# syb0rg/qwen3-tts-jetson

Hardware: AMD Instinct MI355X
Metric: audio frames/sec (12 Hz frames) + RTF, Qwen3-TTS-0.6B batch=1 and batch=8xN (higher is better)
Workload: dtype f16; 1 GPU; configs[1]: Qwen3-TTS-0.6B 1 utterance(s)/GPU x 512 frames, talker+code-predictor+vocoder(full) HIP path, temp 0.9 top-k 50; utterances_per_gpu=1, frames=512, vocoder=full, parallelism=utterance-sharded dp1, weights=local GGUF read

## Files before the change

qwen3-tts-jetson_amd/csrc/persist_cp.hip:

```cpp
#include "persist.h"
#include "persist_dev.h"
#ifdef Q3T_DEV
namespace q3t { __device__ uint64_t *g_selprof = nullptr; }
#define SEL_STAMP(k)                                                                                              \
    do {                                                                                                          \
        if (threadIdx.x == 0 && q3t::g_selprof)                                                                   \
            q3t::g_selprof[((size_t)blockIdx.x * PROF_PH + 440 + ((k) >> 2)) * 4 + ((k) & 3)] = wall_clock64();   \
    } while (0)
#endif
#include "select.h"

#pragma clang fp contract(off)
#include "persist_roles.h"

#ifndef Q3T_CP_SGATE
#define Q3T_CP_SGATE 1
#endif
#ifndef Q3T_CP_GATE
#define Q3T_CP_GATE 1
#endif
#ifndef Q3T_CP_WPUB
#define Q3T_CP_WPUB 1
#endif
#ifndef Q3T_CP_PUT_FIRST
// ... 76 lines not shown
#if Q3T_CP_PAIR
#define CP_TOKENS(pass, ps) for (int ps = (pass) == 1 ? 0 : (pass); ps <= (pass); ++ps)
#else
#define CP_TOKENS(pass, ps) if (const int ps = (pass); true)
#endif
__device__ __forceinline__ int ph_of(int pass, int l, int k) { return pass * PPH + 5 * l + k; }
__device__ __forceinline__ int next_layer(int pass, int l) {
    if (pass + 1 == NPASS && l + 1 == NLC) return -1;
    return (l + 1 < NLC && !(pass == 0 && l + 1 == NLC - 1)) ? l + 1 : 0;
}

__device__ __forceinline__ void role_qkv(Ctx &X) {
    const PersistParams &p = X.p;
    CLds &S = X.S;
    const int i = blockIdx.x - QW, t = threadIdx.x, grp = t >> 4;
    const float temp = p.sel.temperature;
    const bool samp = temp > 0.0f && Q3T_CP_RANGE;
    uint4 wq[4][8];
    float4 nw;
    auto issue_qkv = [&](int l) { qkv_issue<Pol>(S.layers[l].qkv, S.layers[l].attn_norm, i, wq, nw); };
    issue_qkv(0);
    for (int pass = PAIR ? 1 : 0; pass < NPASS; ++pass) {
        for (int l = 0; l < NLC; ++l)
        CP_TOKENS(pass, ps) {
            if (ps >= 1 && l == 0) continue;
            X.use(ps);
            const int ph = ph_of(ps, l, 0);
            float4 x;
            if (l == 0) {
                x = ldf4(p.x_in + 4 * t);
            } else {
                uint32_t u[4];
                PROF(ph, 0);
                wait_in<Pol, 4>(X, p.gx + 4 * t, X.tag(ph_of(ps, l - 1, 4)), u);
                PROF(ph, 1);
                x = f4_of(u);
            }
            qkv_phase<Pol>(X, i, x, wq, nw, ph);
            if (ps < pass && l > 0) continue;
            if (l + 1 < NLC) {
                issue_qkv(l + 1);
            } else if (pass >= 1) {
#pragma unroll
                for (int j = 0; j < 2; ++j) issue_row(S.heads[pass - 1], 32 * i + 16 * j + grp, wq[j]);
                nw = ldf4(p.out_norm + 4 * t);
            } else {
                issue_qkv(1);
            }
        }
        if (pass == 0) continue;
        const int hph = ph_of(pass, NLC, 0);
        uint32_t u[4];
        PROF(hph, 0);
        wait_in<Pol, 4>(X, p.gx + 4 * t, X.tag(ph_of(pass, NLC - 1, 4)), u);
        PROF(hph, 1);
        rms_to_f16(f4_of(u), nw, p.eps, S.xs, S.dscr, nullptr);
        __syncthreads();
        head_rows<2>(X, wq);
        __syncthreads();
        PROF(hph, 3);
        if (t < 64) {
            const float lg = S.outv[t & 31];
            const float sv = samp && Q3T_CP_PREDIV ? lg / temp : lg;
            const float mx = group_max<32>(sv), mn = -group_max<32>(sv > -INFINITY ? -sv : -INFINITY);
            if (t < 32 || (samp && t < 34))
                g_put(t < 32 ? p.glog + 32 * i + t : p.glog + CPV + MMS * i + (t - 32),
                      __float_as_uint(t < 32 ? sv : t == 32 ? mx : mn), X.tag(hph));
            if (t < 32) p.logits[32 * i + t] = lg;
        }
        published<Pol>(X, hph);
        if (pass + 1 < NPASS) issue_qkv(1);
    }
}

__device__ __forceinline__ void role_att(Ctx &X) {
    const PersistParams &p = X.p;
    CLds &S = X.S;
    const int g = blockIdx.x - AW, t = threadIdx.x, lane = t & 63, wave = t >> 6;
    const int pg = t >> 4, li = t & 15;
    const int hb = wave == 0 ? g * 256 : wave == 1 ? g * 256 + D : wave == 2 ? NH * D + g * D : (NH + NKV) * D + g * D;
    const int gi = hb + lane;
    for (int e = t; e < NLC * D; e += 256) {
        S.qn[e / D][e % D] = S.layers[e / D].qn[e % D];
        S.kn[e / D][e % D] = S.layers[e / D].kn[e % D];
    }
    for (int e = t; e < 16 * D; e += 256) S.rope[e / D][e % D] = p.rope[e];
    S.sel.hist[t] = 0u;
// ... 99 lines not shown
                    v16[n] = v16[n + 1] = 0.0f;
                    fma2(pr[n >> 3], ok ? v8[n & 7] : 0.0f, ok ? v8[(n + 1) & 7] : 0.0f, v16[n], v16[n + 1]);
                }
#pragma unroll
                for (int m = 0; m < 8; ++m) {
                    const auto sw = __builtin_amdgcn_permlane16_swap(__float_as_uint(v16[2 * m]), __float_as_uint(v16[2 * m + 1]), false, false);
                    c8[m] = __uint_as_float((uint32_t)sw[0]) + __uint_as_float((uint32_t)sw[1]);
                }
#pragma unroll
                for (int q = 0; q < 4; ++q) {
                    const auto sw = __builtin_amdgcn_permlane32_swap(__float_as_uint(c8[2 * q]), __float_as_uint(c8[2 * q + 1]), false, false);
                    const float av = __uint_as_float((uint32_t)sw[0]) + __uint_as_float((uint32_t)sw[1]);
                    const int n = 4 * q + (lane >> 4);
                    S.ared[wave][n >> 3][li * 8 + (n & 7)] = av;
                }
            }
            __syncthreads();
            if (t < 128) {
                const int h = t / (D / 2), d = 2 * (t % (D / 2));
                const float lsum = (S.wsum[0][h] + S.wsum[1][h]) + (S.wsum[2][h] + S.wsum[3][h]);
                const float a0 = (S.ared[0][h][d] + S.ared[1][h][d]) + (S.ared[2][h][d] + S.ared[3][h][d]);
                const float a1 = (S.ared[0][h][d + 1] + S.ared[1][h][d + 1]) + (S.ared[2][h][d + 1] + S.ared[3][h][d + 1]);
                g_put(p.gattn + g * 128 + t, (uint32_t)f2h(a0 / lsum) | ((uint32_t)f2h(a1 / lsum) << 16), X.tag(ph));
            }
            PROF(ph, 2);
        }
        if (pass == 0) continue;
        const int hph = ph_of(pass, NLC, 0);
        const bool samp = p.sel.temperature > 0.0f;
        constexpr bool RNG = Q3T_CP_RANGE;
        const float u = uniform24(spre.seed, spre.utt, (uint64_t)spre.frame, (uint64_t)pass);
        uint32_t u8[8], mm[2];
        PROF(hph, 0);
        if (Q3T_CP_SGATE) g_gate(p.glog + 8 * t, X.tag(hph), X.c);
        if constexpr (Q3T_POLL16) {
            if (samp && RNG) g_wait16_pair<8, 2>(p.glog + 8 * t, p.glog + CPV + MMS * lane, X.tag(hph), u8, mm, X.c);
            else g_waitc<8>(p.glog + 8 * t, X.tag(hph), u8, X.c);
        } else {
            if (samp && RNG) g_wait_pair<8, 2>(p.glog + 8 * t, p.glog + CPV + MMS * lane, X.tag(hph), u8, mm, X.c);
            else g_wait<8>(p.glog + 8 * t, X.tag(hph), u8, X.c);
        }
        PROF(hph, 1);
        float v[SEL_VPT_MAX];
#pragma unroll
        for (int e = 0; e < SEL_VPT_MAX; ++e) v[e] = e < 8 ? __uint_as_float(u8[e]) : -INFINITY;
        SelectSpec sp = p.sel;
        sp.step = pass - 1;
        int sel;
        if (spre.done >= 0) {
            sel = -1;
        } else if (!samp) {
            sel = sel_argmax(v, CPV, 8, S.sel);
        } else if (!RNG) {
            sel = select_token_pre<SEL_CP>(sp, spre, v, S.sel);
        } else {
            float mx = wave_max(__uint_as_float(mm[0])), mn = -wave_max(-__uint_as_float(mm[1]));
            if constexpr (!Q3T_CP_PREDIV) {
#pragma unroll
                for (int e = 0; e < 8; ++e) v[e] = v[e] / p.sel.temperature;
                mx = mx / p.sel.temperature;
                mn = mn / p.sel.temperature;
            }
            sel = sel_sample_range(v, CPV, 8, p.sel.top_k, u, mx, mn, S.sel);
        }
        S.sel.hist[t] = 0u;
        PROF(hph, 3);
        if (g == 0 && t == 0) {
            if (pass + 1 < NPASS) g_put(p.gtok + pass, (uint32_t)max(sel, 0), X.tag(hph));
            if (sel >= 0) select_commit(sp, 0, sel);
            if (pass + 1 == NPASS) __hip_atomic_store(p.seq, X.seq + 1u, __ATOMIC_RELAXED, __HIP_MEMORY_SCOPE_AGENT);
        }
// ... 23 lines not shown
    };
    issue(0);
    int it = 0;
    for (int pass = PAIR ? 1 : 0; pass < NPASS; ++pass) {
        for (int l = 0; l < NLC; ++l)
        CP_TOKENS(pass, ps) {
            if (ps == 0 && l == NLC - 1) continue;
            X.use(ps);
            const int par = it++ & 1;
            const int ph = ph_of(ps, l, 2);
            if (t < 32) {
                const int row = 32 * i + t;
                float xr;
                if (l == 0 && ps == 0) {
                    xr = p.x_in[row];
                } else if (l == 0) {
                    int tok = p.gs.tok[0];
                    if (pass >= 2) {
                        uint32_t u1[1];
                        g_wait<1>(p.gtok + pass - 1, X.tag(ph_of(pass - 1, NLC, 0)), u1, X.c);
                        tok = min((int)u1[0], p.sel.V - 1);
                    }
                    xr = p.xtab ? p.xtab[((size_t)(pass == 1 ? 0 : VOC + (pass - 2) * CPV) + tok) * H + row]
                                : h2f(S.tabs[pass - 1][(size_t)tok * H + row]);
                } else {
                    uint32_t u1[1];
                    g_wait<1>(p.gx + row, X.tag(ph_of(ps, l - 1, 4)), u1, X.c);
                    xr = __uint_as_float(u1[0]);
                }
                S.xr[t] = xr;
            }
            uint32_t u[4];
            PROF(ph, 0);
            wait_in<Pol, 4>(X, p.gattn + 4 * t, X.tag(ph_of(ps, l, 1)), u);
            PROF(ph, 1);
            *reinterpret_cast<uint4 *>(S.xs + 8 * t) = make_uint4(u[0], u[1], u[2], u[3]);
            wave_lds_sync();
            float acc[8];
#pragma unroll
            for (int j = 0; j < 8; ++j) {
                acc[j] = 0.0f;
#pragma unroll
                for (int tt = 0; tt < 4; ++tt)
                    acc[j] = dot8(wo[j][tt], *reinterpret_cast<const uint4 *>(S.xs + wave * 512 + l16 * 8 + tt * 128), acc[j]);
            }
#pragma unroll
            for (int j = 0; j < 8; ++j) {
                acc[j] = group_sum<16>(acc[j]);
                if (l16 == 0) S.red[par][wave][4 * j + grp4] = acc[j];
            }
            __syncthreads();
            if (t < 32) {
                const float (&rd)[4][32] = S.red[par];
                const float s = rd[0][t] + rd[1][t] + rd[2][t] + rd[3][t];
                g_put(p.gx2 + 32 * i + t, __float_as_uint(S.xr[t] + s), X.tag(ph));
            }
            published<Pol>(X, ph);
            if (ps == pass && next_layer(pass, l) >= 0) issue(next_layer(pass, l));
        }
    }
}

__device__ __forceinline__ void role_gu(Ctx &X) {
    const PersistParams &p = X.p;
    CLds &S = X.S;
    const int i = blockIdx.x - UW, t = threadIdx.x;
    uint4 wg[2][8], wu[2][8];
    float4 nw;
    gu_issue(S.layers[0].gu, S.layers[0].ffn_norm, i, wg, wu, nw);
    for (int pass = PAIR ? 1 : 0; pass < NPASS; ++pass) {
        for (int l = 0; l < NLC; ++l)
        CP_TOKENS(pass, ps) {
            if (ps == 0 && l == NLC - 1) continue;
            X.use(ps);
            const int ph = ph_of(ps, l, 3);
            uint32_t u[4];
            PROF(ph, 0);
            wait_in<Pol, 4>(X, p.gx2 + 4 * t, X.tag(ph_of(ps, l, 2)), u);
            PROF(ph, 1);
            gu_phase<Pol>(X, i, f4_of(u), wg, wu, nw, ph);
            const int nl = ps == pass ? next_layer(pass, l) : -1;
            if (nl >= 0) gu_issue(S.layers[nl].gu, S.layers[nl].ffn_norm, i, wg, wu, nw);
        }
    }
}

__device__ __forceinline__ void role_dn(Ctx &X) {
    const PersistParams &p = X.p;
    CLds &S = X.S;
    const int i = blockIdx.x - DW, t = threadIdx.x;
    const int lo = i * H / ND, n = (i + 1) * H / ND - lo;
    uint4 wd[5][6];
    dn_issue(S.layers[0].down, lo, n, wd);
    int it = 0;
    for (int pass = PAIR ? 1 : 0; pass < NPASS; ++pass) {
        for (int l = 0; l < NLC; ++l)
        CP_TOKENS(pass, ps) {
            if (ps == 0 && l == NLC - 1) continue;
            X.use(ps);
            if (t < n) {
                uint32_t u1[1];
                g_wait<1>(p.gx2 + lo + t, X.tag(ph_of(ps, l, 2)), u1, X.c);
                S.xr[t] = __uint_as_float(u1[0]);
            }
            dn_phase<Pol>(X, lo, n, it++ & 1, wd, ph_of(ps, l, 4));
            const int nl = ps == pass ? next_layer(pass, l) : -1;
            if (nl >= 0) dn_issue(S.layers[nl].down, lo, n, wd);
        }
    }
}

__global__ void __launch_bounds__(256) k_cp_roles(const PersistParams p) {
    extern __shared__ __attribute__((aligned(16))) uint8_t smem[];
    CLds &S = *reinterpret_cast<CLds *>(smem);
    const int t = threadIdx.x, w = blockIdx.x;
    Ctx X{p, p, S, Ctl{p.err, false}, __hip_atomic_load(p.seq, __ATOMIC_RELAXED, __HIP_MEMORY_SCOPE_AGENT)};
#ifdef Q3T_DEV
    if (w == 0 && t == 0) g_selprof = p.prof;
#endif
    if (t < NLC) S.layers[t] = p.L[t];
    if (t < 15) S.heads[t] = p.heads[t];
    if (t < 16) S.tabs[t] = p.gs.tabs[t];
    __syncthreads();
    if (w < AW) role_qkv(X);
    else if (w < OW) role_att(X);
    else if (w < UW) role_o(X);
    else if (w < DW) role_gu(X);
    else role_dn(X);
}

size_t cp_roles_lds() { return std::max(sizeof(CLds), (size_t)96 * 1024); }

}

bool persist_cp_roles_resident(int device) {
    int n_cu = 0, blocks = 0;
    if (hipDeviceGetAttribute(&n_cu, hipDeviceAttributeMultiprocessorCount, device) != hipSuccess || n_cu < G) return false;
    const void *k = reinterpret_cast<const void *>(&k_cp_roles);
    if (hipFuncSetAttribute(k, hipFuncAttributeMaxDynamicSharedMemorySize, (int)cp_roles_lds()) != hipSuccess) return false;
    return hipOccupancyMaxActiveBlocksPerMultiprocessor(&blocks, k, 256, cp_roles_lds()) == hipSuccess && blocks >= 1;
}

bool persist_cp_roles(const PersistParams &p, hipStream_t s) {
    if (!p.L || p.n_layers != NLC || !p.heads || !p.logits || !p.rope || !p.x_in || !p.gs.tok || !p.gs.tabs || !p.qkvtab ||
        !p.gx || p.sel.mode != SEL_CP || p.sel.V != CPV) {
        set_error("persist_cp_roles: bad parameters");
        return false;
    }
    static bool attr = false;
    if (!attr) {
        Q3T_HIP(hipFuncSetAttribute(reinterpret_cast<const void *>(&k_cp_roles), hipFuncAttributeMaxDynamicSharedMemorySize,
                                    (int)cp_roles_lds()));
        attr = true;
    }
    hipLaunchKernelGGL(k_cp_roles, dim3(G), dim3(256), cp_roles_lds(), s, p);
    Q3T_HIP(hipGetLastError());
    return true;
}

}
```

qwen3-tts-jetson_amd/csrc/persist_dev.h:

```cpp
#pragma once
#include "persist.h"

namespace q3t {
namespace pdev {

constexpr unsigned SPIN_LIMIT = 1u << 21;
#ifndef Q3T_POLL_SLEEP
#define Q3T_POLL_SLEEP 1
#endif

template <class V>
__device__ __forceinline__ V ldgv(const void *p) {
    typedef const __attribute__((address_space(1))) V gV;
    return *(gV *)(p);
}
__device__ __forceinline__ uint4 ld16(const void *p) {
    const u32x4_t v = ldgv<u32x4_t>(p);
    return make_uint4(v.x, v.y, v.z, v.w);
}
__device__ __forceinline__ float4 ldf4(const float *p) {
    typedef float f4v __attribute__((ext_vector_type(4)));
    const f4v v = ldgv<f4v>(p);
    return make_float4(v.x, v.y, v.z, v.w);
}
__device__ __forceinline__ uint2 ld8(const void *p) {
    typedef unsigned u2v __attribute__((ext_vector_type(2)));
    const u2v v = ldgv<u2v>(p);
    return make_uint2(v.x, v.y);
}

__device__ __forceinline__ void g_put(uint64_t *p, uint32_t payload, uint32_t tag) {
    __hip_atomic_store(p, ((uint64_t)tag << 32) | payload, __ATOMIC_RELAXED, __HIP_MEMORY_SCOPE_AGENT);
}
__device__ __forceinline__ uint64_t g_ld(const uint64_t *p) {
    return __hip_atomic_load(p, __ATOMIC_RELAXED, __HIP_MEMORY_SCOPE_AGENT);
}
__device__ __forceinline__ uint4 ld16_sc1(const uint16_t *p) {
    uint64_t *q = reinterpret_cast<uint64_t *>(const_cast<uint16_t *>(p));
    const uint64_t a = __hip_atomic_load(q, __ATOMIC_RELAXED, __HIP_MEMORY_SCOPE_AGENT);
    const uint64_t b = __hip_atomic_load(q + 1, __ATOMIC_RELAXED, __HIP_MEMORY_SCOPE_AGENT);
    return make_uint4((uint32_t)a, (uint32_t)(a >> 32), (uint32_t)b, (uint32_t)(b >> 32));
}

struct Ctl {
    unsigned *err;
    bool abort;
};
__device__ __forceinline__ bool give_up(Ctl &c, unsigned &it) {
    if ((++it & 255u) == 0 && (__hip_atomic_load(c.err, __ATOMIC_RELAXED, __HIP_MEMORY_SCOPE_AGENT) != 0u || it >= SPIN_LIMIT)) {
        c.abort = true;
        __hip_atomic_fetch_or(c.err, 1u, __ATOMIC_RELAXED, __HIP_MEMORY_SCOPE_AGENT);
        return true;
    }
    return false;
}

template <int N, int STRIDE = 1, int RUN = 1>
__device__ __forceinline__ void g_wait(const uint64_t *base, uint32_t tag, uint32_t (&out)[N], Ctl &c) {
    uint64_t v[N];
    unsigned it = 0;
    while (true) {
#pragma unroll
        for (int i = 0; i < N; ++i) v[i] = g_ld(base + (i / RUN) * STRIDE + i % RUN);
        bool ok = true;
#pragma unroll
        for (int i = 0; i < N; ++i) ok &= (uint32_t)(v[i] >> 32) == tag;
        if (ok || c.abort) break;
        if (give_up(c, it)) break;
        if constexpr (Q3T_POLL_SLEEP > 0) __builtin_amdgcn_s_sleep(Q3T_POLL_SLEEP);
    }
#pragma unroll
    for (int i = 0; i < N; ++i) out[i] = (uint32_t)v[i];
}

#ifndef Q3T_POLL16
#define Q3T_POLL16 1
#endif
template <int M>
__device__ __forceinline__ void ld16_sc1_batch(const uint64_t *const (&a)[M], u32x4_t (&r)[M]) {
// ... 71 lines not shown
    else g_wait<N>(base, tag, out, c);
}

template <int N, int M>
__device__ __forceinline__ void g_wait_pair(const uint64_t *a, const uint64_t *b, uint32_t tag, uint32_t (&oa)[N], uint32_t (&ob)[M],
                                            Ctl &c) {
    uint64_t v[N + M];
    unsigned it = 0;
    while (true) {
#pragma unroll
        for (int i = 0; i < N; ++i) v[i] = g_ld(a + i);
#pragma unroll
        for (int i = 0; i < M; ++i) v[N + i] = g_ld(b + i);
        bool ok = true;
#pragma unroll
        for (int i = 0; i < N + M; ++i) ok &= (uint32_t)(v[i] >> 32) == tag;
        if (ok || c.abort) break;
        if (give_up(c, it)) break;
        if constexpr (Q3T_POLL_SLEEP > 0) __builtin_amdgcn_s_sleep(Q3T_POLL_SLEEP);
    }
#pragma unroll
    for (int i = 0; i < N; ++i) oa[i] = (uint32_t)v[i];
#pragma unroll
    for (int i = 0; i < M; ++i) ob[i] = (uint32_t)v[N + i];
}

__device__ __forceinline__ void g_gate(const uint64_t *g, uint32_t tag, Ctl &c) {
    if ((threadIdx.x & 63) == 0) {
        unsigned it = 0;
        while (!c.abort && (uint32_t)(g_ld(g) >> 32) != tag) {
            give_up(c, it);
            __builtin_amdgcn_s_sleep(1);
        }
    }
    c.abort = __shfl(c.abort ? 1 : 0, 0) != 0;
}
template <int N, int STRIDE = 1, int RUN = 1>
__device__ __forceinline__ void g_wait_gated(const uint64_t *base, uint32_t tag, uint32_t (&out)[N], Ctl &c) {
    g_gate(base, tag, c);
    g_wait<N, STRIDE, RUN>(base, tag, out, c);
}

#ifndef Q3T_WAVE_SYNC
#define Q3T_WAVE_SYNC 1
#endif
__device__ __forceinline__ void wave_lds_sync() {
    if constexpr (Q3T_WAVE_SYNC) {
        __builtin_amdgcn_s_waitcnt(0xc07f);
        __builtin_amdgcn_wave_barrier();
    } else {
        __syncthreads();
    }
}

__device__ __forceinline__ float4 f4_of(const uint32_t (&u)[4]) {
    return make_float4(__uint_as_float(u[0]), __uint_as_float(u[1]), __uint_as_float(u[2]), __uint_as_float(u[3]));
}


__device__ __forceinline__ double block_sum_d(double v, double *scr) {
    const int lane = threadIdx.x & 63, wave = threadIdx.x >> 6;
    v = wave_sum_d(v);
    if (lane == 0) scr[wave] = v;
    __syncthreads();
    return (scr[0] + scr[1]) + (scr[2] + scr[3]);
}

__device__ __forceinline__ void rms_to_f16(float4 x, float4 w, float eps, uint16_t *xs, double *dscr, float *side) {
    const int t = threadIdx.x;
    double ss = (double)(x.x * x.x) + (double)(x.y * x.y) + (double)(x.z * x.z) + (double)(x.w * x.w);
    ss = block_sum_d(ss, dscr);
    const float scale = 1.0f / sqrtf((float)(ss / 1024) + eps);
    const float y0 = (x.x * scale) * w.x, y1 = (x.y * scale) * w.y, y2 = (x.z * scale) * w.z, y3 = (x.w * scale) * w.w;
// ... 43 lines not shown
```

qwen3-tts-jetson_amd/csrc/persist_roles.h:

```cpp
#pragma once
#include "persist_dev.h"

#pragma clang fp contract(off)

namespace q3t {
namespace prole {
using namespace pdev;

constexpr int H = 1024, NH = 16, NKV = 8, D = 128, QKVN = (NH + 2 * NKV) * D, INTER = 3072;

template <class LDS>
struct RoleCtx {
    const PersistParams &p;
    LDS &S;
    Ctl c;
    unsigned seq;
    __device__ uint32_t tag(int ph) const { return ((seq * 1024u + (unsigned)ph) << 1) | 1u; }
};

#define PROF(ph, k)                                                                                           \
    do {                                                                                                      \
        if (X.p.prof && threadIdx.x == 0 && blockIdx.x < PROF_WG) X.p.prof[((size_t)blockIdx.x * PROF_PH + (ph)) * 4 + (k)] = wall_clock64(); \
    } while (0)

template <class P, int N, class C>
__device__ __forceinline__ void wait_in(C &X, const uint64_t *g, uint32_t tag, uint32_t (&u)[N]) {
    if (P::GATE) g_gate(g, tag, X.c);
    P::template wait<N>(g, tag, u, X.c);
}
template <class P, class C>
__device__ __forceinline__ void published(C &X, int ph) {
    PROF(ph, 2);
    if (P::PUT_FIRST) __syncthreads();
}

__device__ __forceinline__ void issue_row(const uint16_t *W, int row, uint4 (&w)[8]) {
    const uint16_t *r = W + (size_t)row * H + (threadIdx.x & 15) * 8;
#pragma unroll
    for (int tt = 0; tt < 8; ++tt) w[tt] = ld16(r + tt * 128);
}

template <class P>
__device__ __forceinline__ void qkv_issue(const uint16_t *W, const float *norm, int i, uint4 (&wq)[4][8], float4 &nw) {
    const int t = threadIdx.x, grp = t >> 4;
#pragma unroll
    for (int j = 0; j < 4; ++j)
        issue_row(W, 64 * i + (P::WPUB ? 16 * (t >> 6) + 4 * j + (grp & 3) : 16 * j + grp), wq[j]);
    nw = ldf4(norm + 4 * t);
}
template <class P, class C>
__device__ __forceinline__ void qkv_phase(C &X, int i, float4 x, const uint4 (&wq)[4][8], float4 nw, int ph) {
    auto &S = X.S;
    const int t = threadIdx.x, l16 = t & 15, grp = t >> 4;
    rms_to_f16(x, nw, X.p.eps, S.xs, S.dscr, nullptr);
    __syncthreads();
    float acc[4];
#pragma unroll
    for (int j = 0; j < 4; ++j) {
        acc[j] = 0.0f;
#pragma unroll
        for (int tt = 0; tt < 8; ++tt) acc[j] = dot8(wq[j][tt], *reinterpret_cast<const uint4 *>(S.xs + l16 * 8 + tt * 128), acc[j]);
// ... 64 lines not shown
        for (int tt = 0; tt < 4; ++tt) {
            const uint4 xv = *reinterpret_cast<const uint4 *>(S.xs + l16 * 8 + tt * 128);
            a0[j] = dot8(wg[j][tt], xv, a0[j]);
            b0[j] = dot8(wu[j][tt], xv, b0[j]);
        }
#pragma unroll
        for (int tt = 4; tt < 8; ++tt) {
            const uint4 xv = *reinterpret_cast<const uint4 *>(S.xs + l16 * 8 + tt * 128);
            a1[j] = dot8(wg[j][tt], xv, a1[j]);
            b1[j] = dot8(wu[j][tt], xv, b1[j]);
        }
    }
#pragma unroll
    for (int j = 0; j < 2; ++j) {
        const float ga = group_sum<16>(a0[j]) + group_sum<16>(a1[j]);
        const float ub = group_sum<16>(b0[j]) + group_sum<16>(b1[j]);
        if (l16 == 0) S.hs[16 * j + grp] = silu_f(ga) * ub;
    }
    __syncthreads();
    if (t < 16) g_put(X.p.gh + 16 * i + t, (uint32_t)f2h(S.hs[2 * t]) | ((uint32_t)f2h(S.hs[2 * t + 1]) << 16), X.tag(ph));
    published<P>(X, ph);
}

__device__ __forceinline__ void dn_issue(const uint16_t *W, int lo, int n, uint4 (&wd)[5][6]) {
    const int t = threadIdx.x, wave = t >> 6, grp4 = (t & 63) >> 4;
#pragma unroll
    for (int j = 0; j < 5; ++j) {
        const uint16_t *r = W + (size_t)(lo + min(4 * j + grp4, n - 1)) * INTER + wave * 768 + (t & 15) * 8;
#pragma unroll
        for (int tt = 0; tt < 6; ++tt) wd[j][tt] = ld16(r + tt * 128);
    }
}
template <class P, class C>
__device__ __forceinline__ void dn_phase(C &X, int lo, int n, int par, const uint4 (&wd)[5][6], int ph) {
    auto &S = X.S;
    const int t = threadIdx.x, wave = t >> 6, l16 = t & 15, grp4 = (t & 63) >> 4;
    uint32_t u[6];
    PROF(ph, 0);
    wait_in<P, 6>(X, X.p.gh + 6 * t, X.tag(ph - 1), u);
    PROF(ph, 1);
    *reinterpret_cast<uint2 *>(S.xs + 12 * t) = make_uint2(u[0], u[1]);
    *reinterpret_cast<uint2 *>(S.xs + 12 * t + 4) = make_uint2(u[2], u[3]);
    *reinterpret_cast<uint2 *>(S.xs + 12 * t + 8) = make_uint2(u[4], u[5]);
    wave_lds_sync();
    float acc[5];
#pragma unroll
    for (int j = 0; j < 5; ++j) {
        acc[j] = 0.0f;
#pragma unroll
        for (int tt = 0; tt < 6; ++tt)
            acc[j] = dot8(wd[j][tt], *reinterpret_cast<const uint4 *>(S.xs + wave * 768 + l16 * 8 + tt * 128), acc[j]);
    }
#pragma unroll
    for (int j = 0; j < 5; ++j) {
        acc[j] = group_sum<16>(acc[j]);
        if (l16 == 0) S.red[par][wave][4 * j + grp4] = acc[j];
    }
    __syncthreads();
    if (t < n) {
        const float (&rd)[4][32] = S.red[par];
        const float s = rd[0][t] + rd[1][t] + rd[2][t] + rd[3][t];
        g_put(X.p.gx + lo + t, __float_as_uint(S.xr[t] + s), X.tag(ph));
    }
    published<P>(X, ph);
}

}
}
```

qwen3-tts-jetson_amd/csrc/persist_tk.hip:

```cpp
#include "persist.h"
#include "persist_dev.h"
#include "select.h"

#include <algorithm>

#pragma clang fp contract(off)
#include "persist_roles.h"

namespace q3t {

namespace {
using namespace prole;

constexpr int VOC = 3072;
constexpr int R = NH / NKV, CHK = 64, PSLOT = 264, MAXCH = 32;
#ifndef Q3T_TK_WPUB
#define Q3T_TK_WPUB 1
#endif
#ifndef Q3T_TK_HOIST
#define Q3T_TK_HOIST 1
#endif
#ifndef Q3T_TK_PUT_FIRST
#define Q3T_TK_PUT_FIRST 0
#endif
// ... 178 lines not shown
            for (int tt = 0; tt < 4; ++tt) acc[j] = dot8(wo[j][tt], *reinterpret_cast<const uint4 *>(S.xs + l16 * 8 + tt * 128), acc[j]);
        }
#pragma unroll
        for (int j = 0; j < 8; ++j) {
            acc[j] = group_sum<16>(acc[j]);
            if (l16 == 0) S.outv[32 * wave + 4 * j + grp4] = acc[j];
        }
        __syncthreads();
        if (t < 128) g_put(p.gop + (size_t)w * H + 128 * rb + t, __float_as_uint(S.outv[t]), X.tag(ph));
        published<Pol>(X, ph);
        if (l + 1 < nl) issue(l + 1);
    }
}

__device__ __forceinline__ void tk_gu(Ctx &X) {
    const PersistParams &p = X.p;
    TLds &S = X.S;
    const int i = blockIdx.x - UW, t = threadIdx.x, nl = X.nl;
    uint4 wg[2][8], wu[2][8];
    float4 nw;
    gu_issue(S.layers[0].gu, S.layers[0].ffn_norm, i, wg, wu, nw);
    for (int l = 0; l < nl; ++l) {
        const int ph = 5 * l + 3;
        float4 xr;
        if (l == 0) {
            xr = gather_x4(p);
        } else {
            uint32_t u4[4];
            g_waitc<4>(p.gx + 4 * t, X.tag(5 * (l - 1) + 4), u4, X.c);
            xr = f4_of(u4);
        }
        uint32_t u[16];
        PROF(ph, 0);
        g_gate(p.gop + 4 * t, X.tag(5 * l + 2), X.c);
        if constexpr (Q3T_POLL16) g_wait16<4, 4, H>(p.gop + 4 * t, X.tag(5 * l + 2), u, X.c);
        else g_wait<16, H, 4>(p.gop + 4 * t, X.tag(5 * l + 2), u, X.c);
        PROF(ph, 1);
        float x[4];
#pragma unroll
        for (int e = 0; e < 4; ++e) {
            const float s = ((__uint_as_float(u[e]) + __uint_as_float(u[4 + e])) + __uint_as_float(u[8 + e])) + __uint_as_float(u[12 + e]);
            x[e] = (e == 0 ? xr.x : e == 1 ? xr.y : e == 2 ? xr.z : xr.w) + s;
        }
        gu_phase<Pol>(X, i, make_float4(x[0], x[1], x[2], x[3]), wg, wu, nw, ph);
        if (l + 1 < nl) gu_issue(S.layers[l + 1].gu, S.layers[l + 1].ffn_norm, i, wg, wu, nw);
    }
}

__device__ __forceinline__ void tk_dn(Ctx &X) {
    const PersistParams &p = X.p;
    TLds &S = X.S;
    const int i = blockIdx.x - DW, t = threadIdx.x, nl = X.nl;
    const int lo = i * H / ND, n = (i + 1) * H / ND - lo;
    uint4 wd[5][6];
    dn_issue(S.layers[0].down, lo, n, wd);
    for (int l = 0; l < nl; ++l) {
        if (t < n) {
            float xr;
            if (l == 0) {
                xr = layer0_x1(p, lo + t);
            } else {
                uint32_t u1[1];
                g_wait<1>(p.gx + lo + t, X.tag(5 * (l - 1) + 4), u1, X.c);
                xr = __uint_as_float(u1[0]);
            }
            uint32_t uo[4];
            g_wait<4, H>(p.gop + lo + t, X.tag(5 * l + 2), uo, X.c);
            const float s = ((__uint_as_float(uo[0]) + __uint_as_float(uo[1])) + __uint_as_float(uo[2])) + __uint_as_float(uo[3]);
            S.xr[t] = xr + s;
// ... 244 lines not shown
    PROF(hph, 1);
    if (p.sel.mode != SEL_NONE) {
        float v[SEL_VPT_MAX];
#pragma unroll
        for (int e = 0; e < SEL_VPT_MAX; ++e) v[e] = e < VOC / 256 ? __uint_as_float(u[e]) : -INFINITY;
        tok = select_token_pre<SEL_CB0>(p.sel, spre, v, S.sel);
    }
    __syncthreads();
    if (t == 0) {
        if (tok >= 0) select_commit(p.sel, 0, tok);
        if (p.adv_pos && !(p.adv_done && p.adv_done[0] >= 0)) {
            p.adv_pos[0] += 1;
            p.adv_frame[0] += 1;
        }
        __hip_atomic_store(p.seq, X.seq + 1u, __ATOMIC_RELAXED, __HIP_MEMORY_SCOPE_AGENT);
    }
    PROF(hph, 2);
}

__global__ void __launch_bounds__(256, 2) k_tk_roles(const PersistParams p) {
    extern __shared__ __attribute__((aligned(16))) uint8_t smem[];
    TLds &S = *reinterpret_cast<TLds *>(smem);
    const int t = threadIdx.x, w = blockIdx.x;
    Ctx X{{p, S, Ctl{p.err, false}, __hip_atomic_load(p.seq, __ATOMIC_RELAXED, __HIP_MEMORY_SCOPE_AGENT)}, p.pos[0], p.n_layers};
    if (t < p.n_layers) S.layers[t] = p.L[t];
    __syncthreads();
    const int sel_w = AW + 8 * p.roles_split;
    if (w >= OW && w < OW + NO) tk_o(X);
    else if (w >= UW && w < UW + NU) tk_gu(X);
    else if (w >= DW && w < DW + ND) tk_dn(X);
    else if (w < AW) tk_qkv(X);
    else if (w < sel_w) tk_att(X);
    else tk_sel(X);
}

bool tk_covers(int n_ctx) {
    const int nch = (n_ctx + CHK - 1) / CHK;
    return nch <= S_MAX && nch <= MAXCH;
}
const void *const tk_fn = reinterpret_cast<const void *>(&k_tk_roles);

}

bool persist_tk_roles_supported(int n_ctx) { return tk_covers(n_ctx); }

bool persist_tk_roles_resident(int device, int n_ctx) {
    int n_cu = 0, blocks = 0;
    if (hipDeviceGetAttribute(&n_cu, hipDeviceAttributeMultiprocessorCount, device) != hipSuccess || n_cu < 256) return false;
    if (!tk_covers(n_ctx)) return false;
    if (hipFuncSetAttribute(tk_fn, hipFuncAttributeMaxDynamicSharedMemorySize, (int)sizeof(TLds)) != hipSuccess) return false;
    return hipOccupancyMaxActiveBlocksPerMultiprocessor(&blocks, tk_fn, 256, sizeof(TLds)) == hipSuccess && blocks >= 2;
}

bool persist_tk_roles(const PersistParams &p0, hipStream_t s) {
    PersistParams p = p0;
    if (!p.L || p.n_layers <= 0 || p.n_layers > MAXL || !p.head || !p.logits || !p.hidden || !p.pos || !p.rope || !p.kc ||
        !p.vc || !p.gx || (p.gather && !(p.gs.tok && p.gs.tabs && p.gs.frame && p.gs.tr && p.gs.tr_len && p.gs.pad)) ||
        (!p.gather && !p.x_in) || (p.sel.mode != SEL_NONE && (p.sel.mode != SEL_CB0 || p.sel.V != VOC))) {
        set_error("persist_tk_roles: bad parameters");
        return false;
    }
    if (!tk_covers(p.n_ctx)) { set_error("persist_tk_roles: context too long"); return false; }
    static bool attr = false;
    if (!attr) {
        Q3T_HIP(hipFuncSetAttribute(tk_fn, hipFuncAttributeMaxDynamicSharedMemorySize, (int)sizeof(TLds)));
        attr = true;
// ... 9 lines not shown
```

Baseline: 856.7 frames/s.

## Pipeline gate polls in inline asm with adaptive quiet sleep and fused sweep

Replaces the single-lane gate poll followed by a separate wait with a hand-written inline-asm loop. The loop keeps several gate polls in flight, spaced by s_sleep, and once the gate flag matches it immediately issues the 16-byte payload sweep loads. It also adds an adaptive 'quiet' pre-sleep based on the minimum observed poll count, to cut polling traffic on the fabric, and uses it for steady-state waits from pass two onward. The aim is lower handoff latency and less memory contention between persistent role blocks. The risk is extra latency if the learned sleep overshoots, plus fragile inline asm; dev-only poll counters are also added.

```diff
diff --git a/qwen3-tts-jetson_amd/csrc/persist_cp.hip b/qwen3-tts-jetson_amd/csrc/persist_cp.hip
--- a/qwen3-tts-jetson_amd/csrc/persist_cp.hip
+++ b/qwen3-tts-jetson_amd/csrc/persist_cp.hip
@@ -132,7 +132,7 @@
             } else {
                 uint32_t u[4];
                 PROF(ph, 0);
-                wait_in<Pol, 4>(X, p.gx + 4 * t, X.tag(ph_of(ps, l - 1, 4)), u);
+                wait_in<Pol, 4>(X, p.gx + 4 * t, X.tag(ph_of(ps, l - 1, 4)), u, pass >= 2);
                 PROF(ph, 1);
                 x = f4_of(u);
             }
@@ -152,7 +152,7 @@
         const int hph = ph_of(pass, NLC, 0);
         uint32_t u[4];
         PROF(hph, 0);
-        wait_in<Pol, 4>(X, p.gx + 4 * t, X.tag(ph_of(pass, NLC - 1, 4)), u);
+        wait_in<Pol, 4>(X, p.gx + 4 * t, X.tag(ph_of(pass, NLC - 1, 4)), u, pass >= 2);
         PROF(hph, 1);
         rms_to_f16(f4_of(u), nw, p.eps, S.xs, S.dscr, nullptr);
         __syncthreads();
@@ -318,11 +318,14 @@
         const float u = uniform24(spre.seed, spre.utt, (uint64_t)spre.frame, (uint64_t)pass);
         uint32_t u8[8], mm[2];
         PROF(hph, 0);
-        if (Q3T_CP_SGATE) g_gate(p.glog + 8 * t, X.tag(hph), X.c);
-        if constexpr (Q3T_POLL16) {
+        if constexpr (Q3T_POLL16 && Q3T_CP_SGATE) {
+            if (samp && RNG) g_wait16_pair_gated<8, 2>(p.glog + 8 * t, p.glog + CPV + MMS * lane, X.tag(hph), u8, mm, X.c);
+            else g_wait16_gated<1, 8>(p.glog + 8 * t, X.tag(hph), u8, X.c);
+        } else if constexpr (Q3T_POLL16) {
             if (samp && RNG) g_wait16_pair<8, 2>(p.glog + 8 * t, p.glog + CPV + MMS * lane, X.tag(hph), u8, mm, X.c);
             else g_waitc<8>(p.glog + 8 * t, X.tag(hph), u8, X.c);
         } else {
+            if (Q3T_CP_SGATE) g_gate(p.glog + 8 * t, X.tag(hph), X.c);
             if (samp && RNG) g_wait_pair<8, 2>(p.glog + 8 * t, p.glog + CPV + MMS * lane, X.tag(hph), u8, mm, X.c);
             else g_wait<8>(p.glog + 8 * t, X.tag(hph), u8, X.c);
         }
@@ -412,7 +415,7 @@
             }
             uint32_t u[4];
             PROF(ph, 0);
-            wait_in<Pol, 4>(X, p.gattn + 4 * t, X.tag(ph_of(ps, l, 1)), u);
+            wait_in<Pol, 4>(X, p.gattn + 4 * t, X.tag(ph_of(ps, l, 1)), u, pass >= 2);
             PROF(ph, 1);
             *reinterpret_cast<uint4 *>(S.xs + 8 * t) = make_uint4(u[0], u[1], u[2], u[3]);
             wave_lds_sync();
@@ -456,7 +459,7 @@
             const int ph = ph_of(ps, l, 3);
             uint32_t u[4];
             PROF(ph, 0);
-            wait_in<Pol, 4>(X, p.gx2 + 4 * t, X.tag(ph_of(ps, l, 2)), u);
+            wait_in<Pol, 4>(X, p.gx2 + 4 * t, X.tag(ph_of(ps, l, 2)), u, pass >= 2);
             PROF(ph, 1);
             gu_phase<Pol>(X, i, f4_of(u), wg, wu, nw, ph);
             const int nl = ps == pass ? next_layer(pass, l) : -1;
@@ -483,7 +486,7 @@
                 g_wait<1>(p.gx2 + lo + t, X.tag(ph_of(ps, l, 2)), u1, X.c);
                 S.xr[t] = __uint_as_float(u1[0]);
             }
-            dn_phase<Pol>(X, lo, n, it++ & 1, wd, ph_of(ps, l, 4));
+            dn_phase<Pol>(X, lo, n, it++ & 1, wd, ph_of(ps, l, 4), pass >= 2);
             const int nl = ps == pass ? next_layer(pass, l) : -1;
             if (nl >= 0) dn_issue(S.layers[nl].down, lo, n, wd);
         }
@@ -507,6 +510,7 @@
     else if (w < UW) role_o(X);
     else if (w < DW) role_gu(X);
     else role_dn(X);
+    PROF_POLLS();
 }
 
 size_t cp_roles_lds() { return std::max(sizeof(CLds), (size_t)96 * 1024); }
diff --git a/qwen3-tts-jetson_amd/csrc/persist_dev.h b/qwen3-tts-jetson_amd/csrc/persist_dev.h
--- a/qwen3-tts-jetson_amd/csrc/persist_dev.h
+++ b/qwen3-tts-jetson_amd/csrc/persist_dev.h
@@ -45,6 +45,10 @@
 struct Ctl {
     unsigned *err;
     bool abort;
+    unsigned qmin = ~0u;
+#ifdef Q3T_DEV
+    unsigned npoll = 0, nwait = 0;
+#endif
 };
 __device__ __forceinline__ bool give_up(Ctl &c, unsigned &it) {
     if ((++it & 255u) == 0 && (__hip_atomic_load(c.err, __ATOMIC_RELAXED, __HIP_MEMORY_SCOPE_AGENT) != 0u || it >= SPIN_LIMIT)) {
@@ -182,6 +186,10 @@
             give_up(c, it);
             __builtin_amdgcn_s_sleep(1);
         }
+#ifdef Q3T_DEV
+        c.npoll += it + 1;
+        ++c.nwait;
+#endif
     }
     c.abort = __shfl(c.abort ? 1 : 0, 0) != 0;
 }
@@ -189,6 +197,193 @@
 __device__ __forceinline__ void g_wait_gated(const uint64_t *base, uint32_t tag, uint32_t (&out)[N], Ctl &c) {
     g_gate(base, tag, c);
     g_wait<N, STRIDE, RUN>(base, tag, out, c);
+}
+
+#ifndef Q3T_GATE_DEPTH
+#define Q3T_GATE_DEPTH 2
+#endif
+#ifndef Q3T_GATE_SLEEP
+#define Q3T_GATE_SLEEP 4
+#endif
+#ifndef Q3T_GATE_QUIET
+#define Q3T_GATE_QUIET 4
+#endif
+static_assert(Q3T_GATE_DEPTH >= 1 && Q3T_GATE_DEPTH <= 6 && Q3T_GATE_SLEEP >= 1, "gate polls in flight: 1 (g_gate) .. 6");
+constexpr unsigned GATE_BURST = 256;
+#define Q3T_GS_STR2(x) #x
+#define Q3T_GS_STR(x) Q3T_GS_STR2(x)
+#define Q3T_GS_SPACE "s_sleep " Q3T_GS_STR(Q3T_GATE_SLEEP) "\n\t"
+#define Q3T_GS_POLL(k) "global_load_dword %[p" #k "], %[a0], off offset:4 sc1\n\t"
+#define Q3T_GS_STEP(k, vm)                                                                                         \
+    "s_waitcnt vmcnt(" #vm ")\n\t"                                                                                  \
+    "v_cmp_eq_u32_e32 vcc, %[p" #k "], %[tag]\n\t"                                                                  \
+    "s_cbranch_vccnz 1f\n\t"                                                                                        \
+    "s_add_u32 %[cnt], %[cnt], 1\n\t"                                                                               \
+    "s_cmp_ge_u32 %[cnt], %[lim]\n\t"                                                                               \
+    "s_cbranch_scc1 2f\n\t" Q3T_GS_POLL(k) Q3T_GS_SPACE
+#if Q3T_GATE_DEPTH == 2
+#define Q3T_GS_PRO Q3T_GS_POLL(0) Q3T_GS_SPACE Q3T_GS_POLL(1) Q3T_GS_SPACE
+#define Q3T_GS_LOOP Q3T_GS_STEP(0, 1) Q3T_GS_STEP(1, 1)
+#define Q3T_GS_POUT , [p0] "=&v"(gp[0]), [p1] "=&v"(gp[1])
+#elif Q3T_GATE_DEPTH == 3
+#define Q3T_GS_PRO Q3T_GS_POLL(0) Q3T_GS_SPACE Q3T_GS_POLL(1) Q3T_GS_SPACE Q3T_GS_POLL(2) Q3T_GS_SPACE
+#define Q3T_GS_LOOP Q3T_GS_STEP(0, 2) Q3T_GS_STEP(1, 2) Q3T_GS_STEP(2, 2)
+#define Q3T_GS_POUT , [p0] "=&v"(gp[0]), [p1] "=&v"(gp[1]), [p2] "=&v"(gp[2])
+#elif Q3T_GATE_DEPTH == 4
+#define Q3T_GS_PRO Q3T_GS_POLL(0) Q3T_GS_SPACE Q3T_GS_POLL(1) Q3T_GS_SPACE Q3T_GS_POLL(2) Q3T_GS_SPACE Q3T_GS_POLL(3) Q3T_GS_SPACE
+#define Q3T_GS_LOOP Q3T_GS_STEP(0, 3) Q3T_GS_STEP(1, 3) Q3T_GS_STEP(2, 3) Q3T_GS_STEP(3, 3)
+#define Q3T_GS_POUT , [p0] "=&v"(gp[0]), [p1] "=&v"(gp[1]), [p2] "=&v"(gp[2]), [p3] "=&v"(gp[3])
+#elif Q3T_GATE_DEPTH == 5
+#define Q3T_GS_PRO Q3T_GS_POLL(0) Q3T_GS_SPACE Q3T_GS_POLL(1) Q3T_GS_SPACE Q3T_GS_POLL(2) Q3T_GS_SPACE Q3T_GS_POLL(3) Q3T_GS_SPACE Q3T_GS_POLL(4) Q3T_GS_SPACE
+#define Q3T_GS_LOOP Q3T_GS_STEP(0, 4) Q3T_GS_STEP(1, 4) Q3T_GS_STEP(2, 4) Q3T_GS_STEP(3, 4) Q3T_GS_STEP(4, 4)
+#define Q3T_GS_POUT , [p0] "=&v"(gp[0]), [p1] "=&v"(gp[1]), [p2] "=&v"(gp[2]), [p3] "=&v"(gp[3]), [p4] "=&v"(gp[4])
+#elif Q3T_GATE_DEPTH == 6
+#define Q3T_GS_PRO Q3T_GS_POLL(0) Q3T_GS_SPACE Q3T_GS_POLL(1) Q3T_GS_SPACE Q3T_GS_POLL(2) Q3T_GS_SPACE Q3T_GS_POLL(3) Q3T_GS_SPACE Q3T_GS_POLL(4) Q3T_GS_SPACE Q3T_GS_POLL(5) Q3T_GS_SPACE
+#define Q3T_GS_LOOP Q3T_GS_STEP(0, 5) Q3T_GS_STEP(1, 5) Q3T_GS_STEP(2, 5) Q3T_GS_STEP(3, 5) Q3T_GS_STEP(4, 5) Q3T_GS_STEP(5, 5)
+#define Q3T_GS_POUT , [p0] "=&v"(gp[0]), [p1] "=&v"(gp[1]), [p2] "=&v"(gp[2]), [p3] "=&v"(gp[3]), [p4] "=&v"(gp[4]), [p5] "=&v"(gp[5])
+#endif
+#if Q3T_GATE_DEPTH > 1
+#define Q3T_GS_GATE                                                                                                \
+    "s_mov_b64 %[sv], exec\n\t"                                                                                     \
+    "s_mov_b64 exec, 1\n\t"                                                                                         \
+    "s_mov_b32 %[cnt], 0\n\t"                                                                                       \
+    "s_mov_b32 %[fnd], 0\n\t" Q3T_GS_PRO                                                                            \
+    "0:\n\t" Q3T_GS_LOOP                                                                                            \
+    "s_branch 0b\n"                                                                                                 \
+    "1:\n\t"                                                                                                        \
+    "s_mov_b32 %[fnd], 1\n"                                                                                         \
+    "2:\n\t"                                                                                                        \
+    "s_mov_b64 exec, %[sv]\n\t"
+#define Q3T_GS_SWEEP(m) "global_load_dwordx4 %[r" #m "], %[a" #m "], off sc1\n\t"
+#define Q3T_GS_END "s_waitcnt vmcnt(0)"
+#define Q3T_GS_OUT(m) , [r##m] "=&v"(r[m])
+#define Q3T_GS_IN(m) , [a##m] "v"(a[m])
+#define Q3T_GS_HEAD [cnt] "=&s"(cnt), [fnd] "=&s"(fnd), [sv] "=&s"(sv) Q3T_GS_POUT
+#define Q3T_GS_TAIL [tag] "v"(tag), [lim] "s"(GATE_BURST)
+template <int M>
+__device__ __forceinline__ bool gate_sweep16_burst(const uint64_t *const (&a)[M], uint32_t tag, u32x4_t (&r)[M], unsigned &cnt) {
+    uint32_t fnd, gp[Q3T_GATE_DEPTH];
+    uint64_t sv;
+    if constexpr (M == 2)
+        asm volatile(Q3T_GS_GATE Q3T_GS_SWEEP(0) Q3T_GS_SWEEP(1) Q3T_GS_END
+                     : Q3T_GS_HEAD Q3T_GS_OUT(0) Q3T_GS_OUT(1)
+                     : Q3T_GS_TAIL Q3T_GS_IN(0) Q3T_GS_IN(1)
+                     : "memory", "vcc", "scc");
+    else if constexpr (M == 3)
+        asm volatile(Q3T_GS_GATE Q3T_GS_SWEEP(0) Q3T_GS_SWEEP(1) Q3T_GS_SWEEP(2) Q3T_GS_END
+                     : Q3T_GS_HEAD Q3T_GS_OUT(0) Q3T_GS_OUT(1) Q3T_GS_OUT(2)
+                     : Q3T_GS_TAIL Q3T_GS_IN(0) Q3T_GS_IN(1) Q3T_GS_IN(2)
+                     : "memory", "vcc", "scc");
+    else if constexpr (M == 4)
+        asm volatile(Q3T_GS_GATE Q3T_GS_SWEEP(0) Q3T_GS_SWEEP(1) Q3T_GS_SWEEP(2) Q3T_GS_SWEEP(3) Q3T_GS_END
+                     : Q3T_GS_HEAD Q3T_GS_OUT(0) Q3T_GS_OUT(1) Q3T_GS_OUT(2) Q3T_GS_OUT(3)
+                     : Q3T_GS_TAIL Q3T_GS_IN(0) Q3T_GS_IN(1) Q3T_GS_IN(2) Q3T_GS_IN(3)
+                     : "memory", "vcc", "scc");
+    else if constexpr (M == 5)
+        asm volatile(Q3T_GS_GATE Q3T_GS_SWEEP(0) Q3T_GS_SWEEP(1) Q3T_GS_SWEEP(2) Q3T_GS_SWEEP(3) Q3T_GS_SWEEP(4) Q3T_GS_END
+                     : Q3T_GS_HEAD Q3T_GS_OUT(0) Q3T_GS_OUT(1) Q3T_GS_OUT(2) Q3T_GS_OUT(3) Q3T_GS_OUT(4)
+                     : Q3T_GS_TAIL Q3T_GS_IN(0) Q3T_GS_IN(1) Q3T_GS_IN(2) Q3T_GS_IN(3) Q3T_GS_IN(4)
+                     : "memory", "vcc", "scc");
+    else if constexpr (M == 8)
+        asm volatile(Q3T_GS_GATE Q3T_GS_SWEEP(0) Q3T_GS_SWEEP(1) Q3T_GS_SWEEP(2) Q3T_GS_SWEEP(3) Q3T_GS_SWEEP(4) Q3T_GS_SWEEP(5)
+                         Q3T_GS_SWEEP(6) Q3T_GS_SWEEP(7) Q3T_GS_END
+                     : Q3T_GS_HEAD Q3T_GS_OUT(0) Q3T_GS_OUT(1) Q3T_GS_OUT(2) Q3T_GS_OUT(3) Q3T_GS_OUT(4) Q3T_GS_OUT(5) Q3T_GS_OUT(6)
+                           Q3T_GS_OUT(7)
+                     : Q3T_GS_TAIL Q3T_GS_IN(0) Q3T_GS_IN(1) Q3T_GS_IN(2) Q3T_GS_IN(3) Q3T_GS_IN(4) Q3T_GS_IN(5) Q3T_GS_IN(6) Q3T_GS_IN(7)
+                     : "memory", "vcc", "scc");
+    else static_assert(M == 0, "gate_sweep16_burst: unsupported count");
+    return fnd != 0u;
+}
+#endif
+template <int M>
+__device__ __forceinline__ bool gate_sweep16(const uint64_t *const (&a)[M], uint32_t tag, u32x4_t (&r)[M], Ctl &c, bool quiet) {
+#if Q3T_GATE_DEPTH > 1
+    if (__builtin_amdgcn_readfirstlane(c.abort ? 1 : 0) != 0) {
+        c.abort = true;
+        return false;
+    }
+    c.abort = false;
+    unsigned it = 0, q = 0;
+    if constexpr (Q3T_GATE_QUIET > 0) {
+        if (quiet && c.qmin != ~0u) {
+            q = (unsigned)__builtin_amdgcn_readfirstlane((int)c.qmin) * Q3T_GATE_QUIET / 8;
+            for (unsigned i = 0; i < q; ++i) __builtin_amdgcn_s_sleep(Q3T_GATE_SLEEP);
+        }
+    }
+    while (true) {
+        unsigned cnt;
+        if (gate_sweep16_burst<M>(a, tag, r, cnt)) {
+            if constexpr (Q3T_GATE_QUIET > 0)
+                if (quiet) c.qmin = min(c.qmin, q + it + cnt);
+#ifdef Q3T_DEV
+            c.npoll += it + cnt + Q3T_GATE_DEPTH;
+            ++c.nwait;
+#endif
+            break;
+        }
+        it += cnt;
+        if (__hip_atomic_load(c.err, __ATOMIC_RELAXED, __HIP_MEMORY_SCOPE_AGENT) != 0u || it >= SPIN_LIMIT) {
+            c.abort = true;
+            if ((threadIdx.x & 63) == 0) __hip_atomic_fetch_or(c.err, 1u, __ATOMIC_RELAXED, __HIP_MEMORY_SCOPE_AGENT);
+            return false;
+        }
+    }
+    bool ok = true;
+#pragma unroll
+    for (int m = 0; m < M; ++m) ok &= r[m].y == tag && r[m].w == tag;
+    return ok;
+#else
+    return false;
+#endif
+}
+template <int RUNS, int RUN, int STRIDE = 0>
+__device__ __forceinline__ void g_wait16_gated(const uint64_t *base, uint32_t tag, uint32_t (&out)[RUNS * RUN], Ctl &c,
+                                               bool quiet = false) {
+    static_assert(RUN % 2 == 0, "pairs");
+    if constexpr (Q3T_GATE_DEPTH > 1) {
+        constexpr int M = RUNS * RUN / 2;
+        const uint64_t *a[M];
+#pragma unroll
+        for (int k = 0; k < RUNS; ++k)
+#pragma unroll
+            for (int j = 0; j < RUN / 2; ++j) a[k * (RUN / 2) + j] = base + k * STRIDE + 2 * j;
+        u32x4_t r[M];
+        if (gate_sweep16<M>(a, tag, r, c, quiet)) {
+#pragma unroll
+            for (int m = 0; m < M; ++m) {
+                out[2 * m] = r[m].x;
+                out[2 * m + 1] = r[m].z;
+            }
+            return;
+        }
+    } else {
+        g_gate(base, tag, c);
+    }
+    g_wait16<RUNS, RUN, STRIDE>(base, tag, out, c);
+}
+template <int N, int M2>
+__device__ __forceinline__ void g_wait16_pair_gated(const uint64_t *a, const uint64_t *b, uint32_t tag, uint32_t (&oa)[N],
+                                                    uint32_t (&ob)[M2], Ctl &c) {
+    static_assert(N % 2 == 0 && M2 % 2 == 0, "pairs");
+    if constexpr (Q3T_GATE_DEPTH > 1) {
+        constexpr int M = (N + M2) / 2;
+        const uint64_t *ad[M];
+#pragma unroll
+        for (int j = 0; j < N / 2; ++j) ad[j] = a + 2 * j;
+#pragma unroll
+        for (int j = 0; j < M2 / 2; ++j) ad[N / 2 + j] = b + 2 * j;
+        u32x4_t r[M];
+        if (gate_sweep16<M>(ad, tag, r, c, false)) {
+#pragma unroll
+            for (int m = 0; m < N / 2; ++m) { oa[2 * m] = r[m].x; oa[2 * m + 1] = r[m].z; }
+#pragma unroll
+            for (int m = 0; m < M2 / 2; ++m) { ob[2 * m] = r[N / 2 + m].x; ob[2 * m + 1] = r[N / 2 + m].z; }
+            return;
+        }
+    } else {
+        g_gate(a, tag, c);
+    }
+    g_wait16_pair<N, M2>(a, b, tag, oa, ob, c);
 }
 
 #ifndef Q3T_WAVE_SYNC
diff --git a/qwen3-tts-jetson_amd/csrc/persist_roles.h b/qwen3-tts-jetson_amd/csrc/persist_roles.h
--- a/qwen3-tts-jetson_amd/csrc/persist_roles.h
+++ b/qwen3-tts-jetson_amd/csrc/persist_roles.h
@@ -23,10 +23,26 @@
         if (X.p.prof && threadIdx.x == 0 && blockIdx.x < PROF_WG) X.p.prof[((size_t)blockIdx.x * PROF_PH + (ph)) * 4 + (k)] = wall_clock64(); \
     } while (0)
 
+#ifdef Q3T_DEV
+#define PROF_POLLS()                                                                                          \
+    do {                                                                                                      \
+        if (X.p.prof && threadIdx.x == 64 && blockIdx.x < PROF_WG) {                                          \
+            X.p.prof[((size_t)blockIdx.x * PROF_PH + PROF_PH - 1) * 4 + 0] = X.c.npoll;                       \
+            X.p.prof[((size_t)blockIdx.x * PROF_PH + PROF_PH - 1) * 4 + 1] = X.c.nwait;                       \
+        }                                                                                                     \
+    } while (0)
+#else
+#define PROF_POLLS() do { } while (0)
+#endif
+
 template <class P, int N, class C>
-__device__ __forceinline__ void wait_in(C &X, const uint64_t *g, uint32_t tag, uint32_t (&u)[N]) {
-    if (P::GATE) g_gate(g, tag, X.c);
-    P::template wait<N>(g, tag, u, X.c);
+__device__ __forceinline__ void wait_in(C &X, const uint64_t *g, uint32_t tag, uint32_t (&u)[N], bool quiet = true) {
+    if constexpr (P::GATE && Q3T_GATE_DEPTH > 1 && Q3T_POLL16 && N % 2 == 0) {
+        g_wait16_gated<1, N>(g, tag, u, X.c, quiet);
+    } else {
+        if (P::GATE) g_gate(g, tag, X.c);
+        P::template wait<N>(g, tag, u, X.c);
+    }
 }
 template <class P, class C>
 __device__ __forceinline__ void published(C &X, int ph) {
@@ -157,12 +173,12 @@
     }
 }
 template <class P, class C>
-__device__ __forceinline__ void dn_phase(C &X, int lo, int n, int par, const uint4 (&wd)[5][6], int ph) {
+__device__ __forceinline__ void dn_phase(C &X, int lo, int n, int par, const uint4 (&wd)[5][6], int ph, bool quiet = true) {
     auto &S = X.S;
     const int t = threadIdx.x, wave = t >> 6, l16 = t & 15, grp4 = (t & 63) >> 4;
     uint32_t u[6];
     PROF(ph, 0);
-    wait_in<P, 6>(X, X.p.gh + 6 * t, X.tag(ph - 1), u);
+    wait_in<P, 6>(X, X.p.gh + 6 * t, X.tag(ph - 1), u, quiet);
     PROF(ph, 1);
     *reinterpret_cast<uint2 *>(S.xs + 12 * t) = make_uint2(u[0], u[1]);
     *reinterpret_cast<uint2 *>(S.xs + 12 * t + 4) = make_uint2(u[2], u[3]);
diff --git a/qwen3-tts-jetson_amd/csrc/persist_tk.hip b/qwen3-tts-jetson_amd/csrc/persist_tk.hip
--- a/qwen3-tts-jetson_amd/csrc/persist_tk.hip
+++ b/qwen3-tts-jetson_amd/csrc/persist_tk.hip
@@ -234,9 +234,12 @@
         }
         uint32_t u[16];
         PROF(ph, 0);
-        g_gate(p.gop + 4 * t, X.tag(5 * l + 2), X.c);
-        if constexpr (Q3T_POLL16) g_wait16<4, 4, H>(p.gop + 4 * t, X.tag(5 * l + 2), u, X.c);
-        else g_wait<16, H, 4>(p.gop + 4 * t, X.tag(5 * l + 2), u, X.c);
+        if constexpr (Q3T_POLL16) {
+            g_wait16_gated<4, 4, H>(p.gop + 4 * t, X.tag(5 * l + 2), u, X.c, true);
+        } else {
+            g_gate(p.gop + 4 * t, X.tag(5 * l + 2), X.c);
+            g_wait<16, H, 4>(p.gop + 4 * t, X.tag(5 * l + 2), u, X.c);
+        }
         PROF(ph, 1);
         float x[4];
 #pragma unroll
@@ -547,6 +550,7 @@
     else if (w < AW) tk_qkv(X);
     else if (w < sel_w) tk_att(X);
     else tk_sel(X);
+    PROF_POLLS();
 }
 
 bool tk_covers(int n_ctx) {
```

New measurement: 864.9 frames/s, median of 6. No clear change (+1.0%).
